# lucanest/Phyloformer

Measured on AMD Instinct MI355X. Metric: alignments/sec, 60-leaf/500-site LG+GC-like MSAs, Phyloformer forward (pf.ckpt), higher is better.
Workload: dtype f16x3-split MFMA (two fp16 limbs per operand, 3 passes), fp32 accumulate/residual

## Files before the change

### phyloformer_amd/csrc/pf_device.hip.h

```cpp
#pragma once
#include <hip/hip_runtime.h>
#include <stdint.h>

#include "pf_layout.h"

namespace pfk {

typedef float f32x4 __attribute__((ext_vector_type(4)));
typedef float f32x16 __attribute__((ext_vector_type(16)));
#if PF_F16
typedef _Float16 h16_t;
#define PF_MFMA(a, b, c) __builtin_amdgcn_mfma_f32_32x32x16_f16((a), (b), (c), 0, 0, 0)
#define PF_DOT2C "v_dot2c_f32_f16"
#define PF_CVT_PK "v_cvt_pk_f16_f32"
#define PF_NEG1_LO 0x0000bc00u
#define PF_NEG1_HI 0xbc000000u
#else
typedef __bf16 h16_t;
#define PF_MFMA(a, b, c) __builtin_amdgcn_mfma_f32_32x32x16_bf16((a), (b), (c), 0, 0, 0)
#define PF_DOT2C "v_dot2c_f32_bf16"
#define PF_CVT_PK "v_cvt_pk_bf16_f32"
#define PF_NEG1_LO 0x0000bf80u
#define PF_NEG1_HI 0xbf800000u
#endif
// ... 271 lines not shown
    frag_t z;
#pragma unroll
    for (int i = 0; i < 8; ++i) z[i] = (h16_t)0.f;
    return z;
}

#ifndef PF_DEVICE_HELPERS_ONLY
struct MainArgs {
    float* x;
    float* qrow;
    const float* qcol;
    const frag_t* mfrag;
    const float* rq;
    const float* ctx;
    float* spart;
    float* outpart;
    const frag_t* wimg;
    const float* consts;
    const frag_t* wv_lo;
    const float* table;
    const uint8_t* idx;
    const int16_t* pair_i;
    const int16_t* pair_j;
    int B, N, P, Lloc;
    int flat;
    int nt_aln;
    int slots_aln;
    size_t trash_tok;
    int store_x_last;
    unsigned long long* prof;
    int ablate;
};

enum { MODE_FIRST = 0, MODE_MID = 1, MODE_LAST = 2, MODE_MID0 = 3 };

struct TilePos { int b, kt, r0, l0; };
template <bool FLAT>
__device__ __forceinline__ TilePos tile_pos(const MainArgs& a, int task, int ntiles) {
    TilePos q;
    q.b = task / a.nt_aln;
    q.kt = task - q.b * a.nt_aln;
    if (FLAT) { const int tok0 = q.kt * 32; q.r0 = tok0 / a.Lloc; q.l0 = tok0 - q.r0 * a.Lloc; }
    else { q.r0 = q.kt / ntiles; q.l0 = (q.kt - q.r0 * ntiles) * 32; }
    return q;
}
template <bool FLAT>
__device__ __forceinline__ TilePos tile_next(const MainArgs& a, TilePos q) {
    if (++q.kt == a.nt_aln) { q.b++; q.kt = 0; q.r0 = 0; q.l0 = 0; return q; }
    q.l0 += 32;
    if (q.l0 >= a.Lloc) { q.l0 = FLAT ? q.l0 - a.Lloc : 0; q.r0++; }
    return q;
}
struct LanePos { size_t tok0; int toff, l, nvalid, wrap; bool valid, in_r1; };
template <bool FLAT>
__device__ __forceinline__ LanePos lane_pos(const MainArgs& a, const TilePos& q, int t) {
    LanePos o;
    o.tok0 = ((size_t)q.b * a.P + q.r0) * a.Lloc + q.l0;
    const int left = FLAT ? a.P * a.Lloc - q.kt * 32 : a.Lloc - q.l0;
    o.nvalid = min(32, left);
    o.wrap = (FLAT && q.r0 + 1 < a.P) ? min(32, a.Lloc - q.l0) : 32;
    o.valid = t < o.nvalid;
    o.toff = min(t, o.nvalid - 1);
    o.in_r1 = o.toff >= o.wrap;
    o.l = q.l0 + o.toff - (o.in_r1 ? a.Lloc : 0);
    return o;
}
__device__ __forceinline__ void part_range(int flat, int pr, int nparts, int P, int L, int slots_aln, long* first, int* count) {
    if (!flat) { *first = (long)pr * nparts; *count = nparts; return; }
    const int b = pr / P, p = pr - b * P;
    const int k0 = (int)(((long)p * L) >> 5), k1 = (int)((((long)p + 1) * L - 1) >> 5);
    *first = (long)b * slots_aln + k0 + p;
    *count = k1 - k0 + 1;
}

template <int MODE, bool FLAT>
__global__ void __launch_bounds__(MAIN_THREADS, MAIN_WAVES / 4) k_main(MainArgs a) {
    extern __shared__ __attribute__((aligned(16))) unsigned char smem[];
    lds_frag_t lw = (lds_frag_t)smem;
    lds_f32_t lc = (lds_f32_t)(smem + FRAG_END * 16);

    {
        constexpr int lo = (MODE == MODE_FIRST) ? FRAG_WV : 0;
        constexpr int hi = (MODE == MODE_LAST) ? FRAG_WV : FRAG_END;
        static_assert(lo % 64 == 0 && hi % 64 == 0 && FRAG_END % 64 == 0, "the image is copied in whole waves");
        const frag_t* src = a.wimg;
        const int wv = threadIdx.x >> 6, ln = threadIdx.x & 63;
        const float cv = a.consts[min((int)threadIdx.x, CONST_LEN - 1)];
#pragma unroll
        for (int k = 0; k < (hi - lo + MAIN_THREADS - 1) / MAIN_THREADS; ++k) {
            const int f0 = lo + k * MAIN_THREADS + wv * 64;
            if (f0 < hi) __builtin_amdgcn_global_load_lds(src + f0 + ln, smem + (size_t)f0 * 16, 16, 0, 0);
        }
        static_assert(CONST_LEN <= MAIN_THREADS, "one constant per thread");
        if (threadIdx.x < CONST_LEN) reinterpret_cast<float*>(smem + FRAG_END * 16)[threadIdx.x] = cv;
        asm volatile("s_waitcnt vmcnt(0)" ::: "memory");
    }
    __syncthreads();

    const int lane = threadIdx.x & 63;
    const int wave = __builtin_amdgcn_readfirstlane(threadIdx.x >> 6);
    const int t = lane & 31;
    const int h = lane >> 5;
    const int ntiles = (a.Lloc + 31) >> 5;
    const int ntasks = a.B * a.nt_aln;
    if (wave >= MAIN_WAVES / 2) __builtin_amdgcn_s_setprio(1);
    unsigned long long tacc[6] = {0, 0, 0, 0, 0, 0}, tprev = 0;
#define PF_TICK(k) do { if (a.prof) { const unsigned long long tn_ = __builtin_amdgcn_s_memtime(); tacc[k] += tn_ - tprev; tprev = tn_; } } while (0)
    if (a.prof) tprev = __builtin_amdgcn_s_memtime();
    lds_frag_t w1p = lw + FRAG_W1 + lane;
    lds_frag_t w2p = lw + FRAG_W2 + lane;
    lds_frag_t wop = lw + FRAG_WO + lane;
    lds_frag_t qkp = lw + FRAG_QK + h * 8 + (t & 7);
    lds_f32_t lch = lc + 4 * h;
    PF_OPAQUE(wop); PF_OPAQUE(qkp); PF_OPAQUE(lch);
    lds_frag_t wvp = wop + (FRAG_WV - FRAG_WO);

    {
        const int nwaves = gridDim.x * MAIN_WAVES;
#ifndef PF_RUN_MAX
#define PF_RUN_MAX 8
#endif
        const int run = max(1, min(PF_RUN_MAX, ntasks / (nwaves * 8)));
        int run0 = (blockIdx.x * MAIN_WAVES + wave) * run;
        const int task0 = run0, task1 = ntasks;
        TilePos cur = tile_pos<FLAT>(a, min(task0, ntasks - 1), ntiles);
        int frag_row = -1;
        frag_t mfr[4];
        f32x4 rqv = {0.f, 0.f, 0.f, 0.f};
        f32x4 px[8], pctx[8], pqr, pqc;
        int pri = 0, prj = 0;
        auto prefetch = [&](const TilePos& np) {
            const LanePos nl = lane_pos<FLAT>(a, np, t);
            const int ll = nl.l, pb = np.b;
            const size_t tk = nl.tok0 + nl.toff;
            if (MODE == MODE_MID0) {
                const uint8_t* ib = a.idx + (size_t)pb * a.N * a.Lloc + ll;
                const int pp = np.r0 + (nl.in_r1 ? 1 : 0);
                pri = residue(ib[(size_t)a.pair_i[pp] * a.Lloc]);
                prj = residue(ib[(size_t)a.pair_j[pp] * a.Lloc]);
            } else {
                const f32x4* xp = reinterpret_cast<const f32x4*>(a.x + tk * 64 + 4 * h);
#pragma unroll
                for (int g = 0; g < 8; ++g) px[g] = xp[2 * g];
            }
            pqr = *reinterpret_cast<const f32x4*>(a.qrow + tk * 4);
            pqc = *reinterpret_cast<const f32x4*>(a.qcol + tk * 4);
            if (MODE != MODE_FIRST) {
                int hq = h;
// ... 2 lines not shown
#pragma unroll
                for (int g = 0; g < 8; ++g) pctx[g] = cp[2 * g];
            }
        };
        if (MODE != MODE_FIRST && task0 < task1) prefetch(cur);

        for (int task = task0; task < task1;) {
            const int b = cur.b;
            const int row = b * a.P + cur.r0;
            int ntask = task + 1;
            TilePos nxt = tile_next<FLAT>(a, cur);
            if (ntask == run0 + run) {
                run0 += nwaves * run;
                ntask = run0;
                if (ntask < task1) nxt = tile_pos<FLAT>(a, ntask, ntiles);
            }
            const LanePos lp = lane_pos<FLAT>(a, cur, t);
            const bool straddle = lp.wrap < 32;
            int ai = 0, aj = 0;
            if (MODE == MODE_FIRST) { const int pp = cur.r0 + (lp.in_r1 ? 1 : 0); ai = a.pair_i[pp]; aj = a.pair_j[pp]; }
            auto load_mfr = [&](int r) {
                const frag_t* mf = a.mfrag + (size_t)r * 128 + t;
#pragma unroll
                for (int q = 0; q < 4; ++q) mfr[q] = mf[q * 32];
                typedef const f32x4 __attribute__((address_space(4)))* const_f32x4_t;
                rqv = *(const_f32x4_t)(unsigned long long)(a.rq + (size_t)__builtin_amdgcn_readfirstlane(r) * 4);
                frag_row = r;
            };
            if (MODE != MODE_FIRST && row != frag_row) load_mfr(row);
            const bool valid = lp.valid;
            const int lc_ = lp.l;
            const size_t tok = lp.tok0 + lp.toff;
            float x[32];

            if (MODE == MODE_FIRST) {
                const int ri = residue(a.idx[((size_t)b * a.N + ai) * a.Lloc + lc_]);
                const int rj = residue(a.idx[((size_t)b * a.N + aj) * a.Lloc + lc_]);
                const f32x4* ti = reinterpret_cast<const f32x4*>(a.table + ri * 64 + 4 * h);
                const f32x4* tj = reinterpret_cast<const f32x4*>(a.table + rj * 64 + 4 * h);
#pragma unroll
                for (int g = 0; g < 8; ++g) {
                    f32x4 u = ti[2 * g], w = tj[2 * g];
#pragma unroll
                    for (int i = 0; i < 4; ++i) x[4 * g + i] = u[i] + w[i];
                }
            } else {
                if (MODE == MODE_MID0) {
                    const f32x4* ti = reinterpret_cast<const f32x4*>(a.table + pri * 64 + 4 * h);
                    const f32x4* tj = reinterpret_cast<const f32x4*>(a.table + prj * 64 + 4 * h);
#pragma unroll
                    for (int g = 0; g < 8; ++g) {
                        const f32x4 u = ti[2 * g], w = tj[2 * g];
#pragma unroll
                        for (int i = 0; i < 4; ++i) x[4 * g + i] = u[i] + w[i];
                    }
                } else {
#pragma unroll
                    for (int g = 0; g < 8; ++g)
#pragma unroll
                        for (int i = 0; i < 4; ++i) x[4 * g + i] = px[g][i];
                }
                PF_TICK(0);
                if (!(a.ablate & 8)) {
                    f32x16 ya[2];
#pragma unroll
                    for (int j = 0; j < 32; ++j) ya[j >> 4][j & 15] = x[j];
// ... 12 lines not shown
                        };
                        mix(h == 0 && !lp.in_r1);
                        if (straddle) {
                            load_mfr(row + 1);
                            mix(h == 0 && lp.in_r1);
                        }
                    }
                    {
                        const f32x4 qc = pqc * COLAPPLY_B_SCALE;
                        float o[32];
#pragma unroll
                        for (int g = 0; g < 8; ++g) {
                            const f32x4 u = pctx[g];
#pragma unroll
                            for (int i = 0; i < 4; ++i) o[4 * g + i] = u[i] * qc[g >> 1];
                        }
#pragma unroll
                        for (int s = 0; s < 4; ++s) {
                            frag_t ob_hi, ob_lo;
                            split8(&o[8 * s], ob_hi, ob_lo);
#pragma unroll
                            for (int To = 0; To < 2; ++To) {
                                lds_frag_t f = wop + ((To * 4 + s) * 2) * 64;
                                const frag_t a_hi = f[0], a_lo = f[64];
                                mfma3(ya[To], a_hi, a_lo, ob_hi, ob_lo, To == 1);
                            }
                        }
                    }
#pragma unroll
                    for (int j = 0; j < 32; ++j) x[j] = ya[j >> 4][j & 15];
                }

                PF_TICK(1);
                if (!(a.ablate & 16)) {
                    frag_t xb_hi[4], xb_lo[4];
                    {
                        float xn[32];
                        ln_pair(x, xn);
#pragma unroll
                        for (int s = 0; s < 4; ++s) split8(&xn[8 * s], xb_hi[s], xb_lo[s]);
                    }
                    f32x16 oa[2];
                    load_acc_bias(oa[0], lch + CONST_B2);
                    load_acc_bias(oa[1], lch + CONST_B2 + 32);
#pragma unroll
                    for (int j = 0; j < 32; ++j) oa[j >> 4][j & 15] += x[j];
                    if (ntask < task1) prefetch(nxt);
                    PF_TICK(2);
#pragma unroll 1
                    for (int T = 0; T < 8; ++T) {
                        f32x16 ha;
                        lds_frag_t f1 = w1p + T * 512;
                        lds_frag_t f2 = w2p + T * 256;
                        lds_f32_t bp = lch + CONST_B1 + 32 * T;
                        PF_OPAQUE(f1); PF_OPAQUE(f2); PF_OPAQUE(bp);
                        load_acc_bias(ha, bp);
                        frag_t fh = f1[0], fl = f1[64];
#pragma unroll
                        for (int s = 0; s < 4; ++s) {
                            frag_t nh, nl;
                            if (s < 3) { nh = f1[(s + 1) * 128]; nl = f1[(s + 1) * 128 + 64]; }
                            else { nh = f2[0]; nl = f2[64]; }
                            mfma3(ha, fh, fl, xb_hi[s], xb_lo[s]);
                            fh = nh; fl = nl;
                        }
                        frag_t g_hi[2], g_lo[2];
                        gelu_split8(ha, 0, g_hi[0], g_lo[0]);
                        gelu_split8(ha, 8, g_hi[1], g_lo[1]);
#pragma unroll
                        for (int st = 0; st < 4; ++st) {
                            const int u = st >> 1, To = st & 1;
                            frag_t nh = fh, nl = fl;
                            if (st < 3) {
                                const int nu = (st + 1) >> 1, nTo = (st + 1) & 1;
                                nh = f2[(nTo * 32 + nu * 2) * 64];
                                nl = f2[(nTo * 32 + nu * 2) * 64 + 64];
                            }
                            mfma3(oa[To], fh, fl, g_hi[u], g_lo[u], To == 1);
                            fh = nh; fl = nl;
                        }
                    }
                    PF_TICK(3);
#pragma unroll
                    for (int j = 0; j < 32; ++j) x[j] = oa[j >> 4][j & 15];
                }
            }

            if (MODE != MODE_LAST && !(a.ablate & 4)) {
                frag_t wl[8];
#pragma unroll
                for (int i = WVLO_LDS; i < 8; ++i) wl[i] = a.wv_lo[i * 64 + lane];
                __builtin_amdgcn_sched_barrier(0);
                {
                    const size_t stok = valid ? tok : a.trash_tok + t;
                    f32x4* xo = reinterpret_cast<f32x4*>(a.x + stok * 64 + 4 * h);
#pragma unroll
                    for (int g = 0; g < 8; ++g) {
                        f32x4 u = {x[4 * g], x[4 * g + 1], x[4 * g + 2], x[4 * g + 3]};
                        xo[2 * g] = u;
                    }
                }
                if (a.ablate & 32) { cur = nxt; task = ntask; continue; }
                f32x16 va[3];
                {
                    float xn[32];
                    ln_pair(x, xn);
                    frag_t xb_hi[4], xb_lo[4];
#pragma unroll
                    for (int s = 0; s < 4; ++s) split8(&xn[8 * s], xb_hi[s], xb_lo[s]);
#pragma unroll
                    for (int s = 0; s < 4; ++s) {
                        const frag_t q_hi = qkp[(s * 2) * 16], q_lo = qkp[(s * 2 + 1) * 16];
                        if (s == 0) mfma3_zero(va[2], q_hi, q_lo, xb_hi[s], xb_lo[s]);
                        else mfma3(va[2], q_hi, q_lo, xb_hi[s], xb_lo[s]);
                    }
#pragma unroll
                    for (int s = 0; s < 4; ++s)
#pragma unroll
                        for (int T = 0; T < 2; ++T) {
                            const frag_t f_hi = wvp[(T * 4 + s) * 64];
                            const frag_t f_lo = T * 4 + s < WVLO_LDS ? wvp[(FRAG_WVLO - FRAG_WV) + (T * 4 + s) * 64] : wl[T * 4 + s];
// ... 10 lines not shown
                for (int i = 0; i < 4; ++i) ot[i] = pair_other(qk[i], h);
                float qn[4], kn[4];
#pragma unroll
                for (int i = 0; i < 4; ++i) {
                    qn[i] = h ? ot[i] : qk[i];
                    kn[i] = h ? qk[i] : ot[i];
                }
                {
                    const size_t stok = valid ? tok : a.trash_tok + t;
                    f32x4 qs = {qn[0], qn[1], qn[2], qn[3]};
                    *reinterpret_cast<f32x4*>(a.qrow + stok * 4) = qs;
                }
                const long slot0 = (long)b * a.slots_aln + cur.kt + (FLAT ? cur.r0 : 0);
                for (int part = 0; part < (straddle ? 2 : 1); ++part) {
                    float* sp = a.spart + (size_t)(slot0 + part) * SROW;
                    const float vm = (valid && lp.in_r1 == (part == 1)) ? 1.f : 0.f;
                    float km[4];
#pragma unroll
                    for (int i = 0; i < 4; ++i) km[i] = kn[i] * vm;
                    {
                        float qk8[8];
#pragma unroll
                        for (int i = 0; i < 4; ++i) { qk8[i] = vm * qn[i]; qk8[4 + i] = km[i]; }
                        const float sqk = treduce8(qk8, t);
                        if (lane < 8) sp[64 + lane] = sqk;
                    }
                    {
                        float kv[32];
#pragma unroll
                        for (int j = 0; j < 32; ++j) kv[j] = km[j >> 3] * va[j >> 4][j & 15];
                        sp[kmap(t, h)] = treduce32(kv, t);
                    }
                }
            } else if (MODE == MODE_LAST) {
                float z = 0.f;
#pragma unroll
                for (int g = 0; g < 8; ++g) {
                    const f32x4 w4 = *(lds_f32x4_t)(lch + CONST_HW + 8 * g);
#pragma unroll
                    for (int i = 0; i < 4; ++i) z = fmaf(w4[i], x[4 * g + i], z);
                }
                z = pair_sum(z) + lc[CONST_HB];
                const float spz = softplus20(z);
                const long slot0 = (long)b * a.slots_aln + cur.kt + (FLAT ? cur.r0 : 0);
                for (int part = 0; part < (straddle ? 2 : 1); ++part) {
                    const float so = half32_sum((valid && lp.in_r1 == (part == 1)) ? spz : 0.f);
                    if (lane == 0) a.outpart[slot0 + part] = so;
                }
                if (a.store_x_last && valid) {
                    f32x4* xo = reinterpret_cast<f32x4*>(a.x + tok * 64 + 4 * h);
#pragma unroll
                    for (int g = 0; g < 8; ++g) {
                        f32x4 u = {x[4 * g], x[4 * g + 1], x[4 * g + 2], x[4 * g + 3]};
                        xo[2 * g] = u;
                    }
                }
            }
            PF_TICK(4);
            cur = nxt;
            task = ntask;
        }
    }
    if (a.prof && __builtin_amdgcn_mbcnt_hi(~0u, __builtin_amdgcn_mbcnt_lo(~0u, 0u)) == 0) {
#pragma unroll
        for (int k = 0; k < 6; ++k) atomicAdd(a.prof + k, tacc[k]);
    }
#undef PF_TICK
}

constexpr int EMBED_THREADS = 512;
constexpr int EMBED_LDS_BYTES = (PAIRTAB_ROWS * PAIRTAB_W + 22 * 64) * 4;
struct EmbedArgs {
    const uint8_t* idx;
    const int16_t* pair_i;
    const int16_t* pair_j;
    const float* ptab;
    const float* table;
    float* x;
    float* qrow;
    float* srow;
    int B, N, P, Lloc;
    unsigned* bad_idx;
// ... 646 lines not shown
```

### phyloformer_amd/csrc/pf_host_prep.h

```cpp
#pragma once
#include <algorithm>
#include <cmath>
#include <cstdint>
#include <cstring>
#include <vector>

#include "pf_layout.h"

namespace pfhost {
using namespace pfk;

inline uint16_t f2bf(float f) {
    uint32_t u;
    std::memcpy(&u, &f, 4);
    if ((u & 0x7fffffffu) > 0x7f800000u) return uint16_t((u >> 16) | 0x40);
    u += 0x7fffu + ((u >> 16) & 1u);
    return uint16_t(u >> 16);
}
inline float bf2f(uint16_t b) {
    uint32_t u = uint32_t(b) << 16;
    float f;
    std::memcpy(&f, &u, 4);
    return f;
}
// ... 50 lines not shown
                    const size_t base = ((size_t)(T * nS + s) * 2) * 64;
                    out[(base + lane) * 8 + i] = hi;
                    out[(base + 64 + lane) * 8 + i] = lo;
                }
}

inline void pack_qk_frags(const float* wq, const float* wk, uint16_t* qk) {
    for (int s = 0; s < 4; ++s)
        for (int kg = 0; kg < 2; ++kg)
            for (int m = 0; m < 8; ++m)
                for (int i = 0; i < 8; ++i) {
                    const int k = kmap_h(8 * s + i, kg);
                    const float w = (m < 4) ? wq[(size_t)m * E + k] : wk[(size_t)(m - 4) * E + k];
                    const uint16_t hi = f2x(w), lo = f2x(w - x2f(hi));
                    qk[(((size_t)s * 2 + 0) * 16 + kg * 8 + m) * 8 + i] = hi;
                    qk[(((size_t)s * 2 + 1) * 16 + kg * 8 + m) * 8 + i] = lo;
                }
}

inline void pack_row_stats(const float* wv, const float* wq, const float* wk, uint16_t* img_tail ,
                    uint16_t* wv_lo) {
    std::vector<uint16_t> full((size_t)2 * 4 * 2 * 64 * 8);
    pack_frags(wv, E, E, E, full.data());
    for (int T = 0; T < 2; ++T)
        for (int s = 0; s < 4; ++s)
            for (int lane = 0; lane < 64; ++lane)
                for (int i = 0; i < 8; ++i) {
                    const size_t src = (((size_t)(T * 4 + s) * 2) * 64 + lane) * 8 + i;
                    const size_t dst = ((size_t)(T * 4 + s) * 64 + lane) * 8 + i;
                    img_tail[dst] = full[src];
                    wv_lo[dst] = full[src + 64 * 8];
                }
    pack_qk_frags(wq, wk, img_tail + (size_t)(FRAG_QK - FRAG_WV) * 8);
}

struct AttnHost {
    const float *g, *b, *wq, *bq, *wk, *bk, *wv, *bv, *wo, *bo;
};

inline void fold(const float* W, const float* bias, const float* g, const float* beta, int M, int K,
          std::vector<float>& Wf, std::vector<float>& bf) {
    Wf.resize((size_t)M * K);
    bf.resize(M);
    for (int m = 0; m < M; ++m) {
        double acc = bias ? bias[m] : 0.0;
        for (int k = 0; k < K; ++k) {
            Wf[(size_t)m * K + k] = (float)((double)W[(size_t)m * K + k] * (double)g[k]);
            acc += (double)W[(size_t)m * K + k] * (double)beta[k];
        }
        bf[m] = (float)acc;
    }
}

inline void build_pair_table(const float* table, const AttnHost& r, std::vector<float>& out) {
    out.assign((size_t)PAIRTAB_ROWS * PAIRTAB_W, 0.f);
    auto elu1 = [](double z) { return z > 0 ? z + 1.0 : std::exp(z); };
    for (int a = 0; a < NA; ++a)
        for (int b = 0; b < NA; ++b) {
            double x[E], xn[E], mean = 0, var = 0;
            for (int c = 0; c < E; ++c) { x[c] = (double)(table[a * E + c] + table[b * E + c]); mean += x[c]; }
            mean /= E;
            for (int c = 0; c < E; ++c) var += (x[c] - mean) * (x[c] - mean);
            const double rstd = 1.0 / std::sqrt(var / E + (double)LN_EPS);
            for (int c = 0; c < E; ++c) xn[c] = (x[c] - mean) * rstd;
            double q[NH], k[NH];
            for (int hh = 0; hh < NH; ++hh) {
// ... 56 lines not shown
```

### phyloformer_amd/csrc/pf_layout.h

```cpp
#pragma once

#ifndef PF_F16
#define PF_F16 1
#endif

namespace pfk {

constexpr int E = 64;
constexpr int NH = 4;
constexpr int HD = 16;
constexpr int FF = 256;
constexpr int NA = 22;
constexpr int SROW = 72;
constexpr int MROW = 4 * 64;
constexpr float LN_EPS = 1e-5f;

constexpr int FRAG_W1 = 0;
constexpr int FRAG_W2 = FRAG_W1 + 8 * 4 * 2 * 64;
constexpr int FRAG_WO = FRAG_W2 + 2 * 16 * 2 * 64;
constexpr int FRAG_WV = FRAG_WO + 2 * 4 * 2 * 64;
constexpr int FRAG_QK = FRAG_WV + 2 * 4 * 64;
#ifndef PF_WVLO_LDS
#define PF_WVLO_LDS 4
#endif
constexpr int WVLO_LDS = PF_WVLO_LDS;
constexpr int FRAG_WVLO = FRAG_QK + 4 * 2 * 16;
constexpr int FRAG_END = FRAG_WVLO + WVLO_LDS * 64;
constexpr int WVLO_FRAGS = 2 * 4 * 64;
constexpr int CONST_B1 = 0, CONST_B2 = 256, CONST_BQK = 320, CONST_HW = 328, CONST_HB = 392,
              CONST_BOC = 400;
constexpr int CONST_LEN = 464;
constexpr int MAIN_LDS_BYTES = FRAG_END * 16 + CONST_LEN * 4;
constexpr int MFRAG_PER_PAIR = 2 * 2 * 32;

constexpr int MAIN_THREADS = 512;
constexpr int MAIN_WAVES = MAIN_THREADS / 64;

constexpr int PAIRTAB_ROWS = 22 * 22, PAIRTAB_W = 72;

}
```

### phyloformer_amd/csrc/pf_lib.hip

```cpp
#include <hip/hip_runtime.h>
#include <dlfcn.h>

#include <algorithm>
#include <cmath>
#include <cstdarg>
#include <cstdio>
#include <cstdlib>
#include <cstring>
#include <functional>
#include <map>
#include <mutex>
#include <string>
#include <vector>

#include "../../include/phyloformer_amd.h"
#include "pf_device.hip.h"
#include "pf_mha.hip.h"
#include "pf_precise.hip.h"
#include "pf_generic.hip.h"
#include "pf_boot.hip.h"
#include "pf_host_prep.h"

using namespace pfk;
using namespace pfhost;
// ... 91 lines not shown
struct PreciseWeights {
    double* blob = nullptr;
    const double* table = nullptr;
    std::vector<pfp::AttnW> row, col;
    std::vector<pfp::FfnW> ffn;
    const double *hw = nullptr, *hb = nullptr;
};

struct GenericWeights {
    bool ready = false;
    const double* table = nullptr;
    std::vector<pfg::AttnW> row, col;
    std::vector<pfg::FfnW> ffn;
    const double *hw = nullptr, *hb = nullptr;
};

}

struct pf_handle {
    int device = 0;
    int n_blocks = 0;
    hipStream_t stream = nullptr;
    hipStream_t stream2 = nullptr;
    hipStream_t cur = nullptr;
    hipEvent_t ev_fork = nullptr, ev_join = nullptr;
    hipDeviceProp_t prop;
    std::string err;
    int64_t max_seqs = 200;
    bool profile = false;
    bool profile_main_only = false;
    bool debug_keep = false;
    int ablate = 0;
    unsigned long long* phase_prof = nullptr;
    bool force_rccl = false;
    int64_t ws_limit_bytes = (int64_t)24 << 30;
    float* table = nullptr;
    float* pair_table = nullptr;
    bool embed_mfma = false;
    int colstats_fine = -1;
    bool colstats_ring = true;
    bool materialize_x0 = false;
    float* first_consts = nullptr;
    float* first_img = nullptr;
    std::vector<BlockDev> blk;
    std::vector<void*> owned;
    int pair_n = -1;
    int16_t* pair_i = nullptr;
    int16_t* pair_j = nullptr;
    size_t ws_bytes = 0;
    char* ws = nullptr;
    size_t ws2_bytes = 0;
    char* ws2 = nullptr;
    bool overlap = true;
    int reserve_cus = 8;
    uint8_t* d_idx = nullptr; size_t d_idx_bytes = 0;
    float* d_out = nullptr; size_t d_out_bytes = 0;
    uint8_t* d_rep = nullptr; size_t d_rep_bytes = 0;
    void* comm[2] = {nullptr, nullptr};
    int rank = 0, world = 1;
    int64_t coll_calls = 0;
    bool sharded_call = false;
    bool reducing = false;
    bool two_streams = true;
    std::vector<ProfSlot> pending;
    std::vector<hipEvent_t> free_events;
    int64_t prof_n[K_COUNT] = {0};
// ... 168 lines not shown
        if ((rc = upload(h, std::vector<float>(c.bo, c.bo + E), &d.col_bo))) return rc;
        std::vector<float> cwq, cbq, cwk, cbk, cwv, cbv;
        fold(c.wq, c.bq, c.g, c.b, NH, E, cwq, cbq);
        fold(c.wk, c.bk, c.g, c.b, NH, E, cwk, cbk);
        fold(c.wv, c.bv, c.g, c.b, E, E, cwv, cbv);
        f16_note_attn(cwv, cbv, c.wo, true, &ranges);
        std::vector<float> wqk((size_t)8 * E), bqk(8);
        std::copy(cwq.begin(), cwq.end(), wqk.begin());
        std::copy(cwk.begin(), cwk.end(), wqk.begin() + 4 * E);
        for (int i = 0; i < 4; ++i) { bqk[i] = cbq[i]; bqk[4 + i] = cbk[i]; }
        if ((rc = upload(h, wqk, &d.col_wqk))) return rc;
        if ((rc = upload(h, bqk, &d.col_bqk))) return rc;
        std::vector<float> wvT((size_t)E * E);
        for (int hd = 0; hd < E; ++hd)
            for (int cc = 0; cc < E; ++cc) wvT[(size_t)cc * E + hd] = cwv[(size_t)hd * E + cc];
        if ((rc = upload(h, wvT, &d.col_wvT))) return rc;
        if ((rc = upload(h, cbv, &d.col_bv))) return rc;
    }
    for (int k = 0; k < nb; ++k) {
        BlockDev& d = h->blk[k];
        std::vector<float> w1f, b1f;
        fold(ffn[k].w1, ffn[k].b1, ffn[k].g, ffn[k].b, FF, E, w1f, b1f);
        const double alpha = std::sqrt(0.5 * 1.4426950408889634074);
        for (auto& v : w1f) v = (float)((double)v * alpha);
        for (auto& v : b1f) v = (float)((double)v * alpha);
        std::vector<float> w2s((size_t)E * FF);
        for (size_t i = 0; i < w2s.size(); ++i) w2s[i] = (float)((double)ffn[k].w2[i] / alpha * 0.5);
        f16_note_ffn(w1f, b1f, w2s, &ranges);
        std::vector<uint16_t> img((size_t)FRAG_END * 8);
        pack_frags(w1f.data(), FF, E, FF, img.data() + (size_t)FRAG_W1 * 8);
        pack_frags(w2s.data(), E, FF, E, img.data() + (size_t)FRAG_W2 * 8);
        pack_frags(cols[k].wo, E, E, E, img.data() + (size_t)FRAG_WO * 8, COLAPPLY_A_SCALE);
        if (k + 1 < nb) std::copy(row_tail[k + 1].begin(), row_tail[k + 1].end(), img.begin() + (size_t)FRAG_WV * 8);
        if ((rc = upload(h, img, &d.wimg))) return rc;
        std::vector<float> cst(CONST_LEN, 0.f);
        std::copy(b1f.begin(), b1f.end(), cst.begin() + CONST_B1);
        std::copy(ffn[k].b2, ffn[k].b2 + E, cst.begin() + CONST_B2);
        if (k + 1 < nb) std::copy(row_bqk[k + 1].begin(), row_bqk[k + 1].end(), cst.begin() + CONST_BQK);
        std::copy(head_w, head_w + E, cst.begin() + CONST_HW);
        cst[CONST_HB] = head_b[0];
        std::copy(cols[k].bo, cols[k].bo + E, cst.begin() + CONST_BOC);
        if ((rc = upload(h, cst, &d.consts))) return rc;
    }
    std::vector<float> cst0(CONST_LEN, 0.f);
    std::copy(row_bqk[0].begin(), row_bqk[0].end(), cst0.begin() + CONST_BQK);
    std::vector<uint16_t> img0((size_t)FRAG_END * 8, 0);
    std::copy(row_tail[0].begin(), row_tail[0].end(), img0.begin() + (size_t)FRAG_WV * 8);
    check_f16_ranges(h, ranges);
    if ((rc = upload(h, img0, &h->first_img))) return rc;
    return upload(h, cst0, &h->first_consts);
}

int ensure_pairs(pf_handle* h, int N) {
    if (h->pair_n == N) return PF_OK;
    const int P = N * (N - 1) / 2;
    std::vector<int16_t> pi(P), pj(P);
    int k = 0;
    for (int i = 0; i < N; ++i)
        for (int j = i + 1; j < N; ++j) { pi[k] = (int16_t)i; pj[k] = (int16_t)j; ++k; }
    if (h->pair_i) { hipFree(h->pair_i); hipFree(h->pair_j); h->pair_i = h->pair_j = nullptr; }
    HIPCHK(h, hipMalloc((void**)&h->pair_i, P * sizeof(int16_t)));
    HIPCHK(h, hipMalloc((void**)&h->pair_j, P * sizeof(int16_t)));
    HIPCHK(h, hipMemcpyAsync(h->pair_i, pi.data(), P * sizeof(int16_t), hipMemcpyHostToDevice, h->stream));
    HIPCHK(h, hipMemcpyAsync(h->pair_j, pj.data(), P * sizeof(int16_t), hipMemcpyHostToDevice, h->stream));
    HIPCHK(h, hipStreamSynchronize(h->stream));
    h->pair_n = N;
    return PF_OK;
}

size_t align_up(size_t v, size_t a) { return (v + a - 1) / a * a; }

TilePlan tile_plan(const pf_handle* h, int P, int Lloc) { return tile_plan_core(P, Lloc, h->tile_force); }

// ... 105 lines not shown
    return PF_OK;
}

template <int MODE>
int launch_main(pf_handle* h, const MainArgs& a, int kid) {
    const long ntasks = (long)a.B * a.nt_aln;
    const int cus = std::max(1, h->prop.multiProcessorCount - (h->reducing ? h->reserve_cus : 0));
    const int grid = (int)std::max<long>(1, std::min<long>(cus, (ntasks + MAIN_WAVES - 1) / MAIN_WAVES));
    ProfScope ps(h, kid);
    if (a.flat) hipLaunchKernelGGL((k_main<MODE, true>), dim3(grid), dim3(MAIN_THREADS), MAIN_LDS_BYTES, h->cur, a);
    else hipLaunchKernelGGL((k_main<MODE, false>), dim3(grid), dim3(MAIN_THREADS), MAIN_LDS_BYTES, h->cur, a);
    HIPCHK(h, hipGetLastError());
    return PF_OK;
}

struct ShardRun {
    Workspace w;
    const uint8_t* d_idx;
    float* d_out;
    int B, N, P, Lloc, L_total;
    TilePlan tp;
};

MainArgs main_args(pf_handle* h, const ShardRun& r) {
    MainArgs m{};
    m.x = r.w.x; m.qrow = r.w.qrow; m.qcol = r.w.qcol;
    m.mfrag = reinterpret_cast<const frag_t*>(r.w.mfrag); m.rq = r.w.rq; m.ctx = r.w.ctx; m.spart = r.w.spart;
    m.outpart = r.w.outpart; m.table = h->table; m.idx = r.d_idx; m.pair_i = h->pair_i; m.pair_j = h->pair_j;
    m.B = r.B; m.N = r.N; m.P = r.P; m.Lloc = r.Lloc;
    m.flat = r.tp.flat; m.nt_aln = r.tp.nt_aln; m.slots_aln = r.tp.slots_aln;
    m.store_x_last = h->debug_keep ? 1 : 0;
    m.trash_tok = (size_t)r.B * r.P * r.Lloc;
    m.ablate = h->ablate;
    m.prof = h->phase_prof;
    return m;
}

bool x0_on_the_fly(const pf_handle* h) {
    return !h->materialize_x0 && !h->embed_mfma && h->n_blocks > 1;
}

int phase_first(pf_handle* h, const ShardRun& r) {
    int rc;
    if (h->embed_mfma) {
        MainArgs m = main_args(h, r);
        m.wimg = reinterpret_cast<const frag_t*>(h->first_img); m.consts = h->first_consts;
        m.wv_lo = reinterpret_cast<const frag_t*>(h->blk[0].wv_lo);
        rc = launch_main<MODE_FIRST>(h, m, K_EMBED);
        if (rc) return rc;
    } else {
        float* x0 = (x0_on_the_fly(h) && !h->debug_keep) ? nullptr : r.w.x;
        EmbedArgs e{r.d_idx, h->pair_i, h->pair_j, h->pair_table, h->table, x0, r.w.qrow, r.w.srow,
                    r.B, r.N, r.P, r.Lloc, h->bad_idx_dev};
        const int ntasks = r.B * r.P, wpb = EMBED_THREADS / 64;
        const int grid = std::max(1, std::min(h->prop.multiProcessorCount, (ntasks + wpb - 1) / wpb));
        ProfScope ps(h, K_EMBED);
        hipLaunchKernelGGL(k_embed, dim3(grid), dim3(EMBED_THREADS), EMBED_LDS_BYTES, h->cur, e);
        HIPCHK(h, hipGetLastError());
    }
    if (h->debug_keep) return save_tap(h, "x0", r.w.x, (size_t)r.B * r.P * r.Lloc * 64);
    return PF_OK;
}

struct RowStats { const float* p; int nparts; int flat; };

int tiles_of(int Lloc) { return (Lloc + 31) / 32; }

// ... 50 lines not shown
    {
        ColStatsArgs a{w.x, w.qrow, w.mrow, w.qcol, w.part, d.col_wqk, d.col_bqk, d.row_bo, B, P, Lloc, w.G, (Lloc + 31) / 32,
                       w.sub, w.S, w.fine, h->table, r.d_idx, h->pair_i, h->pair_j, r.N};
        ProfScope ps(h, K_COLSTATS);
        const unsigned nblk = (unsigned)(B * a.nchunks * w.nparts());
        if (k == 0 && x0_on_the_fly(h))
            hipLaunchKernelGGL((k_colstats<true, 0, 16>), dim3(nblk), dim3(256), 0, h->cur, a);
        else if (h->colstats_ring)
            hipLaunchKernelGGL((k_colstats<false, PF_CS_RING, PF_CS_MT>), dim3(nblk), dim3(256), 0, h->cur, a);
        else
            hipLaunchKernelGGL((k_colstats<false, 0, 16>), dim3(nblk), dim3(256), 0, h->cur, a);
        HIPCHK(h, hipGetLastError());
    }
    {
        ColFinArgs a{w.part, w.ctx, d.col_wvT, d.col_bv, B, Lloc, w.G, (float)P, P, w.sub, w.S, w.fine};
        ProfScope ps(h, K_COLFIN);
        hipLaunchKernelGGL(k_colfin, dim3(B * Lloc), dim3(COLFIN_THREADS), 0, h->cur, a);
        HIPCHK(h, hipGetLastError());
    }
    if (h->debug_keep) {
        if ((rc = save_tap(h, "ctx" + std::to_string(k), w.ctx, (size_t)B * Lloc * 64))) return rc;
        if ((rc = save_tap(h, "mrow" + std::to_string(k), w.mrow, (size_t)B * P * MROW))) return rc;
    }
    MainArgs m = main_args(h, r);
    m.wimg = reinterpret_cast<const frag_t*>(d.wimg);
    m.consts = d.consts;
    if (k + 1 < h->n_blocks) {
        m.wv_lo = reinterpret_cast<const frag_t*>(h->blk[k + 1].wv_lo);
        if (k == 0 && x0_on_the_fly(h)) rc = launch_main<MODE_MID0>(h, m, K_MAIN);
        else rc = launch_main<MODE_MID>(h, m, K_MAIN);
        if (rc) return rc;
    } else {
        m.wv_lo = nullptr;
        if ((rc = launch_main<MODE_LAST>(h, m, K_MAIN))) return rc;
    }
    if (h->debug_keep && (rc = save_tap(h, "x" + std::to_string(k + 1), w.x, (size_t)B * P * Lloc * 64))) return rc;
    return PF_OK;
}

bool reduces_now(const pf_handle* h) { return h->sharded_call && (h->world > 1 || h->comm[0]); }
bool empty_rank_call(const pf_handle* h, int Lloc) { return Lloc == 0 && reduces_now(h); }

int halves_of(const pf_handle* h, int B) {
    if (B < 2 || h->debug_keep) return 1;
    if (reduces_now(h)) return h->overlap ? 2 : 1;
    return h->two_streams ? 2 : 1;
}

int ensure_second_stream(pf_handle* h) {
    if (h->stream2) return PF_OK;
    HIPCHK(h, hipStreamCreateWithFlags(&h->stream2, hipStreamNonBlocking));
    HIPCHK(h, hipEventCreateWithFlags(&h->ev_fork, hipEventDisableTiming));
    HIPCHK(h, hipEventCreateWithFlags(&h->ev_join, hipEventDisableTiming));
    return PF_OK;
}

struct ForwardScope {
    pf_handle* h;
    ForwardScope(pf_handle* h_, bool reduces) : h(h_) { h->reducing = reduces; }
    ~ForwardScope() { h->cur = h->stream; h->reducing = false; }
};

int forward_chunk(pf_handle* h, const uint8_t* d_idx, int B, int N, int Lloc, int L_total, float* d_out) {
    const int P = N * (N - 1) / 2;
    const bool reduces = reduces_now(h);
    const int nh = halves_of(h, B);
    int rc = ensure_pairs(h, N);
// ... 359 lines not shown
    int ndev = 0;
    hipError_t e = hipGetDeviceCount(&ndev);
    if (e != hipSuccess || ndev == 0)
        return fail(nullptr, PF_EHIP, "no HIP device available (%s); there is no CPU fallback",
                    e != hipSuccess ? hipGetErrorString(e) : "device count is 0");
    if (device < 0 || device >= ndev) return fail(nullptr, PF_EINVAL, "device %d out of range (have %d)", device, ndev);
    pf_handle* h = new pf_handle();
    if (const char* e = getenv("PF_TWO_STREAMS")) h->two_streams = atoi(e) != 0;
    if (getenv("PF_ROW_TILES")) h->tile_force = 0;
    if (getenv("PF_FLAT_TILES")) h->tile_force = 1;
    if (const char* v = getenv("PF_COLSTATS_RING")) h->colstats_ring = atoi(v) != 0;
    h->device = device;
    int rc = PF_OK;
    do {
        if ((e = hipSetDevice(device)) != hipSuccess) { rc = fail(nullptr, PF_EHIP, "hipSetDevice: %s", hipGetErrorString(e)); break; }
        if ((e = hipGetDeviceProperties(&h->prop, device)) != hipSuccess) { rc = fail(nullptr, PF_EHIP, "hipGetDeviceProperties: %s", hipGetErrorString(e)); break; }
        if (std::string(h->prop.gcnArchName).rfind("gfx950", 0) != 0) {
            rc = fail(nullptr, PF_EHIP, "device %d is %s; this library is built for gfx950 only", device, h->prop.gcnArchName);
            break;
        }
        if ((e = hipStreamCreateWithFlags(&h->stream, hipStreamNonBlocking)) != hipSuccess) { rc = fail(nullptr, PF_EHIP, "hipStreamCreate: %s", hipGetErrorString(e)); break; }
        h->cur = h->stream;
        if ((e = hipHostMalloc((void**)&h->bad_idx_host, sizeof(unsigned), hipHostMallocMapped | hipHostMallocCoherent)) != hipSuccess ||
            (e = hipHostGetDevicePointer((void**)&h->bad_idx_dev, h->bad_idx_host, 0)) != hipSuccess) {
            rc = fail(nullptr, PF_EHIP, "hipHostMalloc (residue flag): %s", hipGetErrorString(e));
            break;
        }
        *h->bad_idx_host = 0u;
        const struct { const void* fn; int bytes; } big_lds[] = {
            {reinterpret_cast<const void*>(&k_main<MODE_FIRST, false>), MAIN_LDS_BYTES},
            {reinterpret_cast<const void*>(&k_main<MODE_MID, false>), MAIN_LDS_BYTES},
            {reinterpret_cast<const void*>(&k_main<MODE_MID0, false>), MAIN_LDS_BYTES},
            {reinterpret_cast<const void*>(&k_main<MODE_LAST, false>), MAIN_LDS_BYTES},
            {reinterpret_cast<const void*>(&k_main<MODE_FIRST, true>), MAIN_LDS_BYTES},
            {reinterpret_cast<const void*>(&k_main<MODE_MID, true>), MAIN_LDS_BYTES},
            {reinterpret_cast<const void*>(&k_main<MODE_MID0, true>), MAIN_LDS_BYTES},
            {reinterpret_cast<const void*>(&k_main<MODE_LAST, true>), MAIN_LDS_BYTES},
            {reinterpret_cast<const void*>(&k_embed), EMBED_LDS_BYTES},
        };
        for (const auto& k : big_lds)
            if ((e = hipFuncSetAttribute(k.fn, hipFuncAttributeMaxDynamicSharedMemorySize, k.bytes)) != hipSuccess) {
                rc = fail(nullptr, PF_EHIP, "hipFuncSetAttribute: %s", hipGetErrorString(e));
                break;
            }
        if (rc) break;
    } while (0);
    if (rc) { pf_destroy(h); return rc; }
    *out = h;
    return PF_OK;
}

int pf_create_bare(int device, pf_handle_t** out) {
    if (!out) return fail(nullptr, PF_EINVAL, "null argument");
    *out = nullptr;
    return open_device(device, out);
}

int pf_create(const pf_weights_t* w, int device, pf_handle_t** out) {
    if (!w || !out || !w->blob) return fail(nullptr, PF_EINVAL, "null argument");
    *out = nullptr;
    if (!generic_arch_ok(w))
        return fail(nullptr, PF_EINVAL,
                    "unsupported architecture: n_blocks=%d n_heads=%d embed_dim=%d n_alphabet=%d "
                    "(n_alphabet must be 22, n_blocks 1..64, embed_dim must be 1..256 and divisible by n_heads)",
                    w->n_blocks, w->n_heads, w->embed_dim, w->n_alphabet);
    if (w->blob_len != pf_blob_len(w->n_blocks, w->n_heads, w->embed_dim))
        return fail(nullptr, PF_EINVAL, "weight blob has %llu floats, expected %llu",
                    (unsigned long long)w->blob_len,
                    (unsigned long long)pf_blob_len(w->n_blocks, w->n_heads, w->embed_dim));
    pf_handle* h = nullptr;
// ... 29 lines not shown
    for (void* p : h->owned) hipFree(p);
    if (h->pair_i) hipFree(h->pair_i);
    if (h->pair_j) hipFree(h->pair_j);
    if (h->ws) hipFree(h->ws);
    if (h->ws2) hipFree(h->ws2);
    if (h->wsp) hipFree(h->wsp);
    if (h->stream2) { hipStreamSynchronize(h->stream2); hipStreamDestroy(h->stream2); }
    if (h->ev_fork) hipEventDestroy(h->ev_fork);
    if (h->ev_join) hipEventDestroy(h->ev_join);
    if (h->d_idx) hipFree(h->d_idx);
    if (h->d_out) hipFree(h->d_out);
    if (h->d_rep) hipFree(h->d_rep);
    if (h->stream) hipStreamDestroy(h->stream);
    if (h->bad_idx_host) hipHostFree(h->bad_idx_host);
    delete h;
    return PF_OK;
}

const char* pf_last_error(const pf_handle_t* h) { return h ? h->err.c_str() : g_create_error.c_str(); }

int pf_set_option(pf_handle_t* h, const char* key, int64_t value) {
    if (!h || !key) return PF_EINVAL;
    const std::string k(key);
    if (k == "max_seqs") h->max_seqs = value;
    else if (k == "profile") { drain_profile(h); h->profile = value != 0; h->profile_main_only = value == 2; }
    else if (k == "debug_keep") h->debug_keep = value != 0;
    else if (k == "embed_mfma") h->embed_mfma = value != 0;
    else if (k == "colstats_fine") h->colstats_fine = value < 0 ? -1 : (value != 0);
    else if (k == "materialize_x0") h->materialize_x0 = value != 0;
    else if (k == "overlap") h->overlap = value != 0;
    else if (k == "two_streams") h->two_streams = value != 0;
    else if (k == "reserve_cus") h->reserve_cus = (int)std::max<int64_t>(0, std::min<int64_t>(value, 128));
    else if (k == "ablate") h->ablate = (int)value;
    else if (k == "force_rccl") h->force_rccl = value != 0;
    else if (k == "colstats_ring") h->colstats_ring = value != 0;
    else if (k == "precise") h->precise = value < 0 ? -1 : (value != 0);
    else if (k == "recheck_above") h->recheck_above = value > 0 ? (double)value : 0.0;
    else if (k == "precise_ffn_valu") h->precise_ffn_valu = value != 0;
    else if (k == "generic") {
        if (h->arch_generic && !value)
            return fail(h, PF_EINVAL, "embed_dim %d / n_heads %d runs on the generic kernels only (option generic cannot be 0)",
                        h->garch.E, h->garch.NH);
        h->generic = value != 0;
    }
    else if (k == "phase_prof") {
        if (value && !h->phase_prof) { HIPCHK(h, hipMalloc((void**)&h->phase_prof, 64)); h->owned.push_back(h->phase_prof); }
        if (h->phase_prof) HIPCHK(h, hipMemset(h->phase_prof, 0, 64));
        if (!value) h->phase_prof = nullptr;
    }
    else if (k == "ws_limit_mb") h->ws_limit_bytes = value << 20;
    else return fail(h, PF_EINVAL, "unknown option '%s'", key);
    return PF_OK;
}

int pf_forward(pf_handle_t* h, const uint8_t* idx, int32_t B, int32_t N, int32_t L, float* out) {
    if (!h) return PF_EINVAL;
    return forward_host_impl(h, idx, B, N, 0, L, L, out);
}

int pf_resample_sites_device(pf_handle_t* h, const uint8_t* d_src, int32_t B, int32_t N, int32_t L, int32_t r_begin, int32_t R,
                             uint64_t seed, uint8_t* d_dst) {
    if (!h) return PF_EINVAL;
    if (!d_src || !d_dst) return fail(h, PF_EINVAL, "null buffer");
    if (B < 1 || N < 1 || L < 1 || R < 1 || r_begin < 0)
        return fail(h, PF_EINVAL, "bad dimensions B=%d N=%d L=%d r_begin=%d R=%d", B, N, L, r_begin, R);
    size_t n = 0;
    if (!mul_size((size_t)B, (size_t)R, (size_t)N * L, &n))
        return fail(h, PF_EINVAL, "B=%d x R=%d replicates of %d x %d overflow the address space", B, R, N, L);
    HIPCHK(h, hipSetDevice(h->device));
    return launch_resample(h, d_src, B, N, L, r_begin, R, seed, d_dst);
}

int pf_bootstrap(pf_handle_t* h, const uint8_t* idx, int32_t B, int32_t N, int32_t L, int32_t R, uint64_t seed, float* out) {
    if (!h) return PF_EINVAL;
    return bootstrap_impl(h, idx, B, N, L, R, seed, out);
}

int pf_forward_device(pf_handle_t* h, const uint8_t* d_idx, int32_t B, int32_t N, int32_t L, float* d_out) {
    if (!h) return PF_EINVAL;
    return forward_device_impl(h, d_idx, B, N, 0, L, L, d_out);
}
// ... 392 lines not shown
```

Measured before the change: 542.5.

## Fold the output head into the last block's FFN second matmul

The last block's W2 projection and bias are folded into the linear regression head on the host. This gives a per-hidden-unit vector u and a constant c0, so the final kernel skips the W2 MFMA pass and the residual update. It accumulates gelu(h)·u plus hw·x directly per lane. The W2 weight image is no longer copied to LDS in this mode. It relies on the head being linear in x, and rounding changes because the fold is computed in double and stored as fp32.

```diff
diff --git a/phyloformer_amd/csrc/pf_device.hip.h b/phyloformer_amd/csrc/pf_device.hip.h
--- a/phyloformer_amd/csrc/pf_device.hip.h
+++ b/phyloformer_amd/csrc/pf_device.hip.h
@@ -327,7 +327,7 @@
     int ablate;
 };
 
-enum { MODE_FIRST = 0, MODE_MID = 1, MODE_LAST = 2, MODE_MID0 = 3 };
+enum { MODE_FIRST = 0, MODE_MID = 1, MODE_LAST = 2, MODE_MID0 = 3, MODE_LAST_FOLD = 4 };
 
 struct TilePos { int b, kt, r0, l0; };
 template <bool FLAT>
@@ -368,23 +368,32 @@
     *count = k1 - k0 + 1;
 }
 
+template <int LO, int HI>
+__device__ __forceinline__ void image_to_lds(const frag_t* src, unsigned char* smem) {
+    static_assert(LO % 64 == 0 && HI % 64 == 0, "the image is copied in whole waves");
+    const int wv = threadIdx.x >> 6, ln = threadIdx.x & 63;
+#pragma unroll
+    for (int k = 0; k < (HI - LO + MAIN_THREADS - 1) / MAIN_THREADS; ++k) {
+        const int f0 = LO + k * MAIN_THREADS + wv * 64;
+        if (f0 < HI) __builtin_amdgcn_global_load_lds(src + f0 + ln, smem + (size_t)f0 * 16, 16, 0, 0);
+    }
+}
+
 template <int MODE, bool FLAT>
 __global__ void __launch_bounds__(MAIN_THREADS, MAIN_WAVES / 4) k_main(MainArgs a) {
+    constexpr bool LAST = MODE == MODE_LAST || MODE == MODE_LAST_FOLD;
+    constexpr bool FOLD = MODE == MODE_LAST_FOLD;
     extern __shared__ __attribute__((aligned(16))) unsigned char smem[];
     lds_frag_t lw = (lds_frag_t)smem;
     lds_f32_t lc = (lds_f32_t)(smem + FRAG_END * 16);
 
     {
-        constexpr int lo = (MODE == MODE_FIRST) ? FRAG_WV : 0;
-        constexpr int hi = (MODE == MODE_LAST) ? FRAG_WV : FRAG_END;
-        static_assert(lo % 64 == 0 && hi % 64 == 0 && FRAG_END % 64 == 0, "the image is copied in whole waves");
-        const frag_t* src = a.wimg;
-        const int wv = threadIdx.x >> 6, ln = threadIdx.x & 63;
         const float cv = a.consts[min((int)threadIdx.x, CONST_LEN - 1)];
-#pragma unroll
-        for (int k = 0; k < (hi - lo + MAIN_THREADS - 1) / MAIN_THREADS; ++k) {
-            const int f0 = lo + k * MAIN_THREADS + wv * 64;
-            if (f0 < hi) __builtin_amdgcn_global_load_lds(src + f0 + ln, smem + (size_t)f0 * 16, 16, 0, 0);
+        if (FOLD) {
+            image_to_lds<FRAG_W1, FRAG_W2>(a.wimg, smem);
+            image_to_lds<FRAG_WO, FRAG_U + U_FRAGS>(a.wimg, smem);
+        } else {
+            image_to_lds<(MODE == MODE_FIRST) ? FRAG_WV : 0, LAST ? FRAG_WV : FRAG_END>(a.wimg, smem);
         }
         static_assert(CONST_LEN <= MAIN_THREADS, "one constant per thread");
         if (threadIdx.x < CONST_LEN) reinterpret_cast<float*>(smem + FRAG_END * 16)[threadIdx.x] = cv;
@@ -409,6 +418,7 @@
     lds_f32_t lch = lc + 4 * h;
     PF_OPAQUE(wop); PF_OPAQUE(qkp); PF_OPAQUE(lch);
     lds_frag_t wvp = wop + (FRAG_WV - FRAG_WO);
+    lds_f32_t luh = (lds_f32_t)(smem + FRAG_U * 16) + 16 * h;
 
     {
         const int nwaves = gridDim.x * MAIN_WAVES;
@@ -477,6 +487,7 @@
             const int lc_ = lp.l;
             const size_t tok = lp.tok0 + lp.toff;
             float x[32];
+            float zh[4] = {0.f, 0.f, 0.f, 0.f};
 
             if (MODE == MODE_FIRST) {
                 const int ri = residue(a.idx[((size_t)b * a.N + ai) * a.Lloc + lc_]);
@@ -555,7 +566,49 @@
                 }
 
                 PF_TICK(1);
-                if (!(a.ablate & 16)) {
+                if (FOLD) {
+#pragma unroll
+                    for (int g = 0; g < 8; ++g) {
+                        const f32x4 w4 = *(lds_f32x4_t)(lch + CONST_HW + 8 * g);
+#pragma unroll
+                        for (int i = 0; i < 4; ++i) zh[i] = fmaf(w4[i], x[4 * g + i], zh[i]);
+                    }
+                }
+                if (FOLD && !(a.ablate & 16)) {
+                    frag_t xb_hi[4], xb_lo[4];
+                    {
+                        float xn[32];
+                        ln_pair(x, xn);
+#pragma unroll
+                        for (int s = 0; s < 4; ++s) split8(&xn[8 * s], xb_hi[s], xb_lo[s]);
+                    }
+                    if (ntask < task1) prefetch(nxt);
+                    PF_TICK(2);
+#pragma unroll 1
+                    for (int T = 0; T < 8; ++T) {
+                        f32x16 ha;
+                        lds_frag_t f1 = w1p + T * 512;
+                        lds_f32_t bp = lch + CONST_B1 + 32 * T;
+                        lds_f32_t up = luh + 32 * T;
+                        PF_OPAQUE(f1); PF_OPAQUE(bp); PF_OPAQUE(up);
+                        load_acc_bias(ha, bp);
+                        frag_t fh = f1[0], fl = f1[64];
+#pragma unroll
+                        for (int s = 0; s < 4; ++s) {
+                            frag_t nh = fh, nl = fl;
+                            if (s < 3) { nh = f1[(s + 1) * 128]; nl = f1[(s + 1) * 128 + 64]; }
+                            mfma3(ha, fh, fl, xb_hi[s], xb_lo[s]);
+                            fh = nh; fl = nl;
+                        }
+#pragma unroll
+                        for (int q = 0; q < 4; ++q) {
+                            const f32x4 u4 = *(lds_f32x4_t)(up + 4 * q);
+#pragma unroll
+                            for (int i = 0; i < 4; ++i) zh[i] = fmaf(u4[i], gelu_scaled(ha[4 * q + i]), zh[i]);
+                        }
+                    }
+                    PF_TICK(3);
+                } else if (!(a.ablate & 16)) {
                     frag_t xb_hi[4], xb_lo[4];
                     {
                         float xn[32];
@@ -609,7 +662,7 @@
                 }
             }
 
-            if (MODE != MODE_LAST && !(a.ablate & 4)) {
+            if (!LAST && !(a.ablate & 4)) {
                 frag_t wl[8];
 #pragma unroll
                 for (int i = WVLO_LDS; i < 8; ++i) wl[i] = a.wv_lo[i * 64 + lane];
@@ -686,22 +739,26 @@
                         sp[kmap(t, h)] = treduce32(kv, t);
                     }
                 }
-            } else if (MODE == MODE_LAST) {
+            } else if (LAST) {
                 float z = 0.f;
-#pragma unroll
-                for (int g = 0; g < 8; ++g) {
-                    const f32x4 w4 = *(lds_f32x4_t)(lch + CONST_HW + 8 * g);
-#pragma unroll
-                    for (int i = 0; i < 4; ++i) z = fmaf(w4[i], x[4 * g + i], z);
-                }
-                z = pair_sum(z) + lc[CONST_HB];
+                if (FOLD) {
+                    z = pair_sum((zh[0] + zh[1]) + (zh[2] + zh[3])) + lc[CONST_C0];
+                } else {
+#pragma unroll
+                    for (int g = 0; g < 8; ++g) {
+                        const f32x4 w4 = *(lds_f32x4_t)(lch + CONST_HW + 8 * g);
+#pragma unroll
+                        for (int i = 0; i < 4; ++i) z = fmaf(w4[i], x[4 * g + i], z);
+                    }
+                    z = pair_sum(z) + lc[CONST_HB];
+                }
                 const float spz = softplus20(z);
                 const long slot0 = (long)b * a.slots_aln + cur.kt + (FLAT ? cur.r0 : 0);
                 for (int part = 0; part < (straddle ? 2 : 1); ++part) {
                     const float so = half32_sum((valid && lp.in_r1 == (part == 1)) ? spz : 0.f);
                     if (lane == 0) a.outpart[slot0 + part] = so;
                 }
-                if (a.store_x_last && valid) {
+                if (!FOLD && a.store_x_last && valid) {
                     f32x4* xo = reinterpret_cast<f32x4*>(a.x + tok * 64 + 4 * h);
 #pragma unroll
                     for (int g = 0; g < 8; ++g) {
diff --git a/phyloformer_amd/csrc/pf_host_prep.h b/phyloformer_amd/csrc/pf_host_prep.h
--- a/phyloformer_amd/csrc/pf_host_prep.h
+++ b/phyloformer_amd/csrc/pf_host_prep.h
@@ -106,6 +106,21 @@
                     wv_lo[dst] = full[src + 64 * 8];
                 }
     pack_qk_frags(wq, wk, img_tail + (size_t)(FRAG_QK - FRAG_WV) * 8);
+}
+
+inline void fold_head(const float* w2 , const float* b2, const float* hw, float hb, double w2_scale,
+                      float* u_img , float* c0) {
+    for (int T = 0; T < FF / 32; ++T)
+        for (int h = 0; h < 2; ++h)
+            for (int r = 0; r < 16; ++r) {
+                const int k = 32 * T + kmap_h(r, h);
+                double acc = 0.0;
+                for (int c = 0; c < E; ++c) acc += (double)hw[c] * (double)w2[(size_t)c * FF + k];
+                u_img[(T * 2 + h) * 16 + r] = (float)(acc * w2_scale);
+            }
+    double acc = (double)hb;
+    for (int c = 0; c < E; ++c) acc += (double)hw[c] * (double)b2[c];
+    *c0 = (float)acc;
 }
 
 struct AttnHost {
diff --git a/phyloformer_amd/csrc/pf_layout.h b/phyloformer_amd/csrc/pf_layout.h
--- a/phyloformer_amd/csrc/pf_layout.h
+++ b/phyloformer_amd/csrc/pf_layout.h
@@ -26,9 +26,12 @@
 constexpr int WVLO_LDS = PF_WVLO_LDS;
 constexpr int FRAG_WVLO = FRAG_QK + 4 * 2 * 16;
 constexpr int FRAG_END = FRAG_WVLO + WVLO_LDS * 64;
+constexpr int FRAG_U = FRAG_WV;
+constexpr int U_FRAGS = FF * 4 / 16;
+static_assert(FRAG_U + U_FRAGS <= FRAG_END, "the folded head fits the last block's tail");
 constexpr int WVLO_FRAGS = 2 * 4 * 64;
 constexpr int CONST_B1 = 0, CONST_B2 = 256, CONST_BQK = 320, CONST_HW = 328, CONST_HB = 392,
-              CONST_BOC = 400;
+              CONST_C0 = 393, CONST_BOC = 400;
 constexpr int CONST_LEN = 464;
 constexpr int MAIN_LDS_BYTES = FRAG_END * 16 + CONST_LEN * 4;
 constexpr int MFRAG_PER_PAIR = 2 * 2 * 32;
diff --git a/phyloformer_amd/csrc/pf_lib.hip b/phyloformer_amd/csrc/pf_lib.hip
--- a/phyloformer_amd/csrc/pf_lib.hip
+++ b/phyloformer_amd/csrc/pf_lib.hip
@@ -147,6 +147,8 @@
     bool debug_keep = false;
     int ablate = 0;
     unsigned long long* phase_prof = nullptr;
+    bool phase_prof_last = false;
+    bool head_fold = true;
     bool force_rccl = false;
     int64_t ws_limit_bytes = (int64_t)24 << 30;
     float* table = nullptr;
@@ -381,6 +383,12 @@
         pack_frags(w2s.data(), E, FF, E, img.data() + (size_t)FRAG_W2 * 8);
         pack_frags(cols[k].wo, E, E, E, img.data() + (size_t)FRAG_WO * 8, COLAPPLY_A_SCALE);
         if (k + 1 < nb) std::copy(row_tail[k + 1].begin(), row_tail[k + 1].end(), img.begin() + (size_t)FRAG_WV * 8);
+        float c0 = 0.f;
+        if (k + 1 == nb) {
+            float u[FF];
+            fold_head(ffn[k].w2, ffn[k].b2, head_w, head_b[0], 1.0 / alpha * 0.5, u, &c0);
+            std::memcpy(img.data() + (size_t)FRAG_U * 8, u, sizeof(u));
+        }
         if ((rc = upload(h, img, &d.wimg))) return rc;
         std::vector<float> cst(CONST_LEN, 0.f);
         std::copy(b1f.begin(), b1f.end(), cst.begin() + CONST_B1);
@@ -388,6 +396,7 @@
         if (k + 1 < nb) std::copy(row_bqk[k + 1].begin(), row_bqk[k + 1].end(), cst.begin() + CONST_BQK);
         std::copy(head_w, head_w + E, cst.begin() + CONST_HW);
         cst[CONST_HB] = head_b[0];
+        cst[CONST_C0] = c0;
         std::copy(cols[k].bo, cols[k].bo + E, cst.begin() + CONST_BOC);
         if ((rc = upload(h, cst, &d.consts))) return rc;
     }
@@ -559,7 +568,7 @@
     m.store_x_last = h->debug_keep ? 1 : 0;
     m.trash_tok = (size_t)r.B * r.P * r.Lloc;
     m.ablate = h->ablate;
-    m.prof = h->phase_prof;
+    m.prof = h->phase_prof_last ? nullptr : h->phase_prof;
     return m;
 }
 
@@ -676,7 +685,18 @@
         if (rc) return rc;
     } else {
         m.wv_lo = nullptr;
-        if ((rc = launch_main<MODE_LAST>(h, m, K_MAIN))) return rc;
+        if (h->phase_prof_last) m.prof = h->phase_prof;
+        if (!h->head_fold) {
+            if ((rc = launch_main<MODE_LAST>(h, m, K_MAIN))) return rc;
+        } else {
+            if ((rc = launch_main<MODE_LAST_FOLD>(h, m, K_MAIN))) return rc;
+            if (h->debug_keep) {
+                MainArgs md = m;
+                md.outpart = w.spart;
+                md.prof = nullptr;
+                if ((rc = launch_main<MODE_LAST>(h, md, K_MAIN))) return rc;
+            }
+        }
     }
     if (h->debug_keep && (rc = save_tap(h, "x" + std::to_string(k + 1), w.x, (size_t)B * P * Lloc * 64))) return rc;
     return PF_OK;
@@ -1102,10 +1122,12 @@
             {reinterpret_cast<const void*>(&k_main<MODE_MID, false>), MAIN_LDS_BYTES},
             {reinterpret_cast<const void*>(&k_main<MODE_MID0, false>), MAIN_LDS_BYTES},
             {reinterpret_cast<const void*>(&k_main<MODE_LAST, false>), MAIN_LDS_BYTES},
+            {reinterpret_cast<const void*>(&k_main<MODE_LAST_FOLD, false>), MAIN_LDS_BYTES},
             {reinterpret_cast<const void*>(&k_main<MODE_FIRST, true>), MAIN_LDS_BYTES},
             {reinterpret_cast<const void*>(&k_main<MODE_MID, true>), MAIN_LDS_BYTES},
             {reinterpret_cast<const void*>(&k_main<MODE_MID0, true>), MAIN_LDS_BYTES},
             {reinterpret_cast<const void*>(&k_main<MODE_LAST, true>), MAIN_LDS_BYTES},
+            {reinterpret_cast<const void*>(&k_main<MODE_LAST_FOLD, true>), MAIN_LDS_BYTES},
             {reinterpret_cast<const void*>(&k_embed), EMBED_LDS_BYTES},
         };
         for (const auto& k : big_lds)
@@ -1201,6 +1223,7 @@
     else if (k == "two_streams") h->two_streams = value != 0;
     else if (k == "reserve_cus") h->reserve_cus = (int)std::max<int64_t>(0, std::min<int64_t>(value, 128));
     else if (k == "ablate") h->ablate = (int)value;
+    else if (k == "head_fold") h->head_fold = value != 0;
     else if (k == "force_rccl") h->force_rccl = value != 0;
     else if (k == "colstats_ring") h->colstats_ring = value != 0;
     else if (k == "precise") h->precise = value < 0 ? -1 : (value != 0);
@@ -1216,6 +1239,7 @@
         if (value && !h->phase_prof) { HIPCHK(h, hipMalloc((void**)&h->phase_prof, 64)); h->owned.push_back(h->phase_prof); }
         if (h->phase_prof) HIPCHK(h, hipMemset(h->phase_prof, 0, 64));
         if (!value) h->phase_prof = nullptr;
+        h->phase_prof_last = value == 2;
     }
     else if (k == "ws_limit_mb") h->ws_limit_bytes = value << 20;
     else return fail(h, PF_EINVAL, "unknown option '%s'", key);
```

Result: faster. 558.3, median of 6 (+2.9%).
